# qitianwu/DIFFormer

Hardware: AMD Instinct MI355X
Metric: DIFFormer-layer forward nodes/sec (higher is better)
Workload: dtype f32; 1 GPU; ogbn-proteins-s; nodes=132534, csr_entries=79255038, in_channels=8, hidden=64, heads=1, layers=4, kernel=simple, use_graph=True, parallelism=single GPU, exact_fp32=False, csr=warm (cached), launch=eager

## Files before the change

### difformer_amd/csrc/gcn_sliced.hip

```cpp
#include <stdlib.h>
#include "dif_common.h"

namespace {

using dif::f32x4;

#ifndef DIF_SLICED_TILE_ROWS
#define DIF_SLICED_TILE_ROWS 10208
#endif
#ifndef DIF_SLICED_MAX_WAVES
#define DIF_SLICED_MAX_WAVES 16
#endif
#ifndef DIF_SLICED_WG_PER_CU
#define DIF_SLICED_WG_PER_CU 1
#endif
constexpr int kSteps = 8;
constexpr int kTileRowsMax = DIF_SLICED_TILE_ROWS;
constexpr int kLdsRows = kTileRowsMax + 16;
constexpr int kWgPerCU = DIF_SLICED_WG_PER_CU;
constexpr int kMaxRounds = 10;
constexpr int kMaxWaves = DIF_SLICED_MAX_WAVES;
constexpr int kGroupCap = 65535;

__device__ const uint8_t kLaneOf[64] = {
    0,  1,  2,  3,  12, 13, 14, 15, 20, 21, 22, 23, 24, 25, 26, 27,
    4,  5,  6,  7,  8,  9,  10, 11, 16, 17, 18, 19, 28, 29, 30, 31,
    32, 33, 34, 35, 44, 45, 46, 47, 52, 53, 54, 55, 56, 57, 58, 59,
    36, 37, 38, 39, 40, 41, 42, 43, 48, 49, 50, 51, 60, 61, 62, 63};

struct Plan {
    int slices, panels, G, PW, W, R, T, NT;
    int S = 1;
};
constexpr int kMaxSplits = 8;

__host__ __device__ __forceinline__ int64_t slot_of(int j, int pw, int PW) {
    return static_cast<int64_t>(j) * PW + ((j & 1) ? PW - 1 - pw : pw);
}

int make_plan(int64_t n_src, int64_t n_rows, int F, Plan& p) {
    if (n_src <= 0 || n_rows <= 0 || F <= 0 || F % 4 != 0 || F / 4 > 256) return DIF_E_SHAPE;
    p.slices = F / 4;
    const int64_t G = (n_rows + 63) / 64;
    int64_t panels = dif::kCUs * kWgPerCU / p.slices;
    if (panels < 1) panels = 1;
    const int64_t cap = static_cast<int64_t>(kMaxWaves) * kMaxRounds;
    if (panels * cap < G) panels = (G + cap - 1) / cap;
    const int64_t nt0 = (n_src + kTileRowsMax - 1) / kTileRowsMax;
    const int64_t need = (G + (cap - kMaxWaves) - 1) / (cap - kMaxWaves);
    int S = 1;
    while (S * 2 <= kMaxSplits && n_src + (n_src >> 4) >= int64_t(2) * S * n_rows && need * S * 2 <= panels && nt0 >= S * 2) S *= 2;
    p.S = S;
    panels /= S;
    if (panels > G) panels = G;
    if (panels * p.slices > (int64_t(1) << 20) || G >= (int64_t(1) << 30)) return DIF_E_RANGE;
    p.panels = static_cast<int>(panels);
    p.G = static_cast<int>(G);
    int bestW = 0, bestR = 1 << 30;
    int64_t bestWaste = int64_t(1) << 60;
    for (int W = kMaxWaves; W >= 1; --W) {
        const int64_t pw = panels * W;
        if (pw > G && W > 1) continue;
        const int R = static_cast<int>((G + pw - 1) / pw);
        const int64_t waste = static_cast<int64_t>(R) * pw - G;
        if (R < bestR || (R == bestR && waste < bestWaste)) { bestW = W; bestR = R; bestWaste = waste; }
    }
    if (bestR > kMaxRounds) return DIF_E_SHAPE;
    p.W = bestW;
    p.R = bestR;
    p.PW = p.panels * p.W;
    const int64_t nt = (nt0 + S - 1) / S * S;
    if (nt > 32767) return DIF_E_RANGE;
    p.NT = static_cast<int>(nt);
    p.T = static_cast<int>((((n_src + nt - 1) / nt) + 15) / 16 * 16);
    return 0;
}

__device__ __forceinline__ void group_bounds(const int32_t* __restrict__ rowptr, const int32_t* __restrict__ blkptr,
                                             int64_t n_src, int NT, int64_t row, int t, int32_t& e0, int32_t& e1) {
    if (NT == 1) { e0 = rowptr[row]; e1 = rowptr[row + 1]; }
    else { e0 = blkptr[static_cast<int64_t>(t) * n_src + row]; e1 = blkptr[static_cast<int64_t>(t + 1) * n_src + row]; }
}

__device__ __forceinline__ void position_bounds(const int32_t* __restrict__ rowptr, const int32_t* __restrict__ blkptr,
                                                int64_t n_src, int NT, int64_t row_begin, const int32_t* __restrict__ order,
                                                const uint16_t* __restrict__ parts, int64_t pos, int t, int32_t& e0,
                                                int32_t& e1) {
    const int64_t lrow = order ? order[pos] : pos;
    if (lrow < 0) { e0 = e1 = 0; return; }
    group_bounds(rowptr, blkptr, n_src, NT, row_begin + lrow, t, e0, e1);
    if (parts) {
        const uint32_t pp = parts[pos];
        const int64_t p = pp & 0xffu, P = pp >> 8, c = e1 - e0;
        e1 = e0 + static_cast<int32_t>(c * (p + 1) / P);
        e0 = e0 + static_cast<int32_t>(c * p / P);
    }
}

struct Counts { uint64_t w[4]; };

__device__ __forceinline__ Counts bucket_starts(const Counts& c) {
    const uint64_t ones = 0x0001000100010001ull;
    Counts s;
    uint64_t carry = 0;
#pragma unroll
    for (int k = 0; k < 4; ++k) {
        const uint64_t inc = c.w[k] * ones;
        s.w[k] = inc - c.w[k] + carry * ones;
        carry += inc >> 48;
    }
    return s;
}

__device__ __forceinline__ uint32_t lane16(const Counts& c, uint32_t q) {
    const uint64_t w = (q < 8u) ? ((q < 4u) ? c.w[0] : c.w[1]) : ((q < 12u) ? c.w[2] : c.w[3]);
    return static_cast<uint32_t>(w >> ((q & 3u) * 16u)) & 0xffffu;
}

__device__ __forceinline__ void bump16(Counts& c, uint32_t q) {
    const uint64_t one = 1ull << ((q & 3u) * 16u);
    const uint32_t k = q >> 2;
    c.w[0] += (k == 0u) ? one : 0ull;
    c.w[1] += (k == 1u) ? one : 0ull;
    c.w[2] += (k == 2u) ? one : 0ull;
    c.w[3] += (k == 3u) ? one : 0ull;
}

__device__ __forceinline__ Counts load_counts(const uint4* __restrict__ cnt, int64_t idx) {
    const uint4 a = cnt[idx * 2], b = cnt[idx * 2 + 1];
    Counts c;
    c.w[0] = static_cast<uint64_t>(a.x) | (static_cast<uint64_t>(a.y) << 32);
    c.w[1] = static_cast<uint64_t>(a.z) | (static_cast<uint64_t>(a.w) << 32);
    c.w[2] = static_cast<uint64_t>(b.x) | (static_cast<uint64_t>(b.y) << 32);
    c.w[3] = static_cast<uint64_t>(b.z) | (static_cast<uint64_t>(b.w) << 32);
    return c;
}

__global__ __launch_bounds__(256) void sliced_sort_kernel(const int32_t* __restrict__ rowptr, const int32_t* __restrict__ blkptr,
                                                          const int32_t* __restrict__ src, int64_t n_src, int NT, int T,
                                                          int64_t row_begin, int64_t n_pos, const int32_t* __restrict__ order,
                                                          const uint16_t* __restrict__ parts,
                                                          uint16_t* __restrict__ srt, uint4* __restrict__ cnt,
                                                          int32_t* __restrict__ status) {
    const int lane = threadIdx.x & 63;
    const int64_t pos = static_cast<int64_t>(blockIdx.x) * 4 + (threadIdx.x >> 6);
    if (pos >= n_pos) return;
    const uint64_t below = (lane == 0) ? 0ull : (~0ull >> (64 - lane));
    uint32_t* cnt32 = reinterpret_cast<uint32_t*>(cnt);
    for (int t = 0; t < NT; ++t) {
        int32_t e0, e1;
        position_bounds(rowptr, blkptr, n_src, NT, row_begin, order, parts, pos, t, e0, e1);
        e0 = __builtin_amdgcn_readfirstlane(e0);
        e1 = __builtin_amdgcn_readfirstlane(e1);
        const int32_t base = t * T;
        if (e1 - e0 > kGroupCap) {
            if (lane == 0) atomicOr(status, 1);
            e1 = e0;
        }
        uint32_t count[16];
#pragma unroll
        for (int q = 0; q < 16; ++q) count[q] = 0;
        for (int32_t c0 = e0; c0 < e1; c0 += 64) {
            const int32_t e = c0 + lane;
            const bool ok = e < e1;
            const uint32_t q = ok ? (static_cast<uint32_t>(src[e] - base) & 15u) : 16u;
#pragma unroll
            for (int qq = 0; qq < 16; ++qq) count[qq] += static_cast<uint32_t>(__popcll(__ballot(q == static_cast<uint32_t>(qq))));
        }
        uint32_t word = 0;
#pragma unroll
        for (int j = 0; j < 8; ++j)
            if (lane == j) word = count[2 * j] | (count[2 * j + 1] << 16);
        if (lane < 8) cnt32[(pos * NT + t) * 8 + lane] = word;
        uint32_t run[16];
        uint32_t acc = 0;
#pragma unroll
        for (int q = 0; q < 16; ++q) { run[q] = acc; acc += count[q]; }
        for (int32_t c0 = e0; c0 < e1; c0 += 64) {
            const int32_t e = c0 + lane;
            const bool ok = e < e1;
            const uint32_t loc = ok ? static_cast<uint32_t>(src[e] - base) : 0u;
            const uint32_t q = ok ? (loc & 15u) : 16u;
            uint32_t dst = 0;
#pragma unroll
            for (int qq = 0; qq < 16; ++qq) {
                const uint64_t m = __ballot(q == static_cast<uint32_t>(qq));
                if (q == static_cast<uint32_t>(qq)) dst = run[qq] + static_cast<uint32_t>(__popcll(m & below));
                run[qq] += static_cast<uint32_t>(__popcll(m));
            }
            if (ok) srt[e0 + dst] = static_cast<uint16_t>(loc);
        }
    }
}

constexpr int kColorThreads = 64;

template <bool EMIT>
__global__ __launch_bounds__(kColorThreads) void sliced_color_kernel(int64_t n_pos, Plan pl, int cap,
                                                                     const uint4* __restrict__ cnt,
                                                                     int32_t* __restrict__ len,
                                                                     const int32_t* __restrict__ tab,
                                                                     uint16_t* __restrict__ ell) {
    const int64_t gid = static_cast<int64_t>(blockIdx.x) * kColorThreads + threadIdx.x;
    const int64_t n_groups = static_cast<int64_t>(pl.G) * pl.NT * 4;
    if (gid >= n_groups) return;
    const int grp = static_cast<int>(gid & 3);
    const int t = static_cast<int>((gid >> 2) % pl.NT);
    const int64_t g = (gid >> 2) / pl.NT;
    const bool packed = cap > 1;
    uint32_t c[16][8];
    uint32_t col[16];
    int rem[16];
    int remaining = 0;
#pragma unroll
    for (int q = 0; q < 16; ++q) col[q] = 0;
#pragma unroll
    for (int i = 0; i < 16; ++i) {
        const int64_t pos = g * 64 + kLaneOf[grp * 16 + i];
        Counts cc = {{0, 0, 0, 0}};
        if (pos < n_pos) cc = load_counts(cnt, pos * pl.NT + t);
        rem[i] = 0;
#pragma unroll
        for (int k = 0; k < 4; ++k) {
            c[i][2 * k] = static_cast<uint32_t>(cc.w[k]);
            c[i][2 * k + 1] = static_cast<uint32_t>(cc.w[k] >> 32);
            const uint32_t q0 = cc.w[k] & 0xffffu, q1 = (cc.w[k] >> 16) & 0xffffu, q2 = (cc.w[k] >> 32) & 0xffffu,
                           q3 = static_cast<uint32_t>(cc.w[k] >> 48);
            col[4 * k] += q0; col[4 * k + 1] += q1; col[4 * k + 2] += q2; col[4 * k + 3] += q3;
            rem[i] += static_cast<int>(q0 + q1 + q2 + q3);
        }
        remaining += rem[i];
    }
    int target = 0;
    if (packed) {
        int longest = 0;
        uint32_t fullest = 0;
#pragma unroll
        for (int i = 0; i < 16; ++i) { longest = max(longest, rem[i]); fullest = max(fullest, col[i]); }
        target = max(longest, static_cast<int>((fullest + cap - 1) / cap));
        target = max(target, __shfl_xor(target, 1));
        target = max(target, __shfl_xor(target, 2));
        target = (target + kSteps - 1) / kSteps * kSteps;
    }
    const int j = static_cast<int>(g / pl.PW);
    const int idxp = static_cast<int>(g % pl.PW);
    const int pw = (j & 1) ? pl.PW - 1 - idxp : idxp;
    const int p = pw % pl.panels, w = pw / pl.panels;
    const int32_t* tb = nullptr;
    int64_t blk0 = 0;
    int nbj = 0;
    if (EMIT) {
        tb = tab + ((static_cast<int64_t>(p) * pl.NT + t) * pl.W + w) * (pl.R + 1);
        blk0 = tb[0];
        nbj = tb[1 + j];
    }
    int64_t rowbase = 0;
    auto record_at = [&](int step) -> uint4* {
        return reinterpret_cast<uint4*>(ell) + (blk0 + rowbase + j) * 64 + grp * kSteps + (step % kSteps);
    };
    auto new_row = [&](int step) {
        if (EMIT && (step % kSteps) == 0) {
            const int k = step / kSteps;
            rowbase = 0;
            for (int j2 = 0; j2 < pl.R; ++j2) { const int v = tb[1 + j2]; rowbase += v < k ? v : k; }
        }
    };
    int step = 0;
    while (remaining > 0) {
        new_row(step);
        uint32_t used = 0, full = 0, picked = 0, qlo = 0, qhi = 0;
        const int start = step & 15;
        const int left = target - step;
#pragma unroll
        for (int pass = 0; pass < 2; ++pass) {
#pragma unroll
            for (int i = 0; i < 16; ++i) {
                if ((i >= start) != (pass == 0)) continue;
                uint32_t key = 0, kshare = 0, kany = 0;
#pragma unroll
                for (int k = 0; k < 8; ++k) {
                    const uint32_t olo = c[i][k] & 0xffffu, ohi = c[i][k] >> 16;
                    const uint32_t wlo = packed ? col[2 * k] : olo, whi = packed ? col[2 * k + 1] : ohi;
                    const uint32_t lo = olo ? ((wlo << 4) | static_cast<uint32_t>(15 - 2 * k)) : 0u;
                    const uint32_t hi = ohi ? ((whi << 4) | static_cast<uint32_t>(14 - 2 * k)) : 0u;
                    const bool ulo = (used >> (2 * k)) & 1u, uhi = (used >> (2 * k + 1)) & 1u;
                    key = max(key, max(ulo ? 0u : lo, uhi ? 0u : hi));
                    if (packed) {
                        const uint32_t slo = (ulo && !((full >> (2 * k)) & 1u)) ? lo : 0u;
                        const uint32_t shi = (uhi && !((full >> (2 * k + 1)) & 1u)) ? hi : 0u;
                        kany = max(kany, max(slo, shi));
                        kshare = max(kshare, max(static_cast<int>(col[2 * k]) >= left ? slo : 0u,
                                                 static_cast<int>(col[2 * k + 1]) >= left ? shi : 0u));
                    }
                }
                bool share = false;
                if (packed) {
                    if (kshare > key) { key = kshare; share = true; }
                    else if (key < 16u && rem[i] >= left && kany >= 16u) { key = kany; share = true; }
                }
                if (key < 16u) continue;
                const uint32_t best = 15u - (key & 15u);
                if (share) full |= 1u << best;
                else used |= 1u << best;
                picked |= 1u << i;
                const uint32_t dec = 1u << (16u * (best & 1u)), wsel = best >> 1;
#pragma unroll
                for (int k = 0; k < 8; ++k) c[i][k] -= (wsel == static_cast<uint32_t>(k)) ? dec : 0u;
#pragma unroll
                for (int q = 0; q < 16; ++q) col[q] -= (best == static_cast<uint32_t>(q)) ? 1u : 0u;
                --rem[i];
                --remaining;
                if (EMIT) {
                    if (i < 8) qlo |= best << (4 * i);
                    else qhi |= best << (4 * (i - 8));
                }
            }
        }
        if (EMIT) {
#pragma unroll
            for (int i = 0; i < 16; ++i) {
                if ((picked >> i) & 1u) continue;
                const uint32_t fq = __builtin_ctz(~used & 0xffffu);
                used |= 1u << fq;
                if (i < 8) qlo |= fq << (4 * i);
                else qhi |= fq << (4 * (i - 8));
            }
            *record_at(step) = uint4{qlo, qhi, picked, 0u};
        }
        ++step;
    }
    if (!EMIT) {
        len[gid] = step;
    } else {
        for (; step < nbj * kSteps; ++step) {
            new_row(step);
            *record_at(step) = uint4{0x76543210u, 0xfedcba98u, 0u, 0u};
        }
    }
}

constexpr int kFillStage = 4096;

template <bool STAGED>
__device__ __forceinline__ void fill_blocks(const uint16_t* __restrict__ mine, const uint16_t* stage, Counts next,
                                            const int32_t* __restrict__ tb, int R, int j, int nbj, int64_t blk0, int grp,
                                            int i, int lane, uint32_t T, uint4* __restrict__ ell) {
    uint64_t n0 = next.w[0], n1 = next.w[1], n2 = next.w[2], n3 = next.w[3];
    const uint32_t himask = (i >= 8) ? ~0u : 0u, sh = 4u * (i & 7);
    for (int k = 0; k < nbj; ++k) {
        int64_t rowbase = 0;
        for (int j2 = 0; j2 < R; ++j2) { const int v = tb[1 + j2]; rowbase += v < k ? v : k; }
        uint4* blk = ell + (blk0 + rowbase + j) * 64;
        uint4 rec[kSteps];
#pragma unroll
        for (int s8 = 0; s8 < kSteps; ++s8) rec[s8] = blk[grp * kSteps + s8];
        uint32_t ent[kSteps];
#pragma unroll
        for (int s8 = 0; s8 < kSteps; ++s8) {
            const uint32_t q = ((((rec[s8].x & ~himask) | (rec[s8].y & himask)) >> sh)) & 15u;
            const bool real = (rec[s8].z >> i) & 1u;
            const uint32_t k = q >> 2;
            const uint64_t m0 = k == 0u ? ~0ull : 0ull, m1 = k == 1u ? ~0ull : 0ull, m2 = k == 2u ? ~0ull : 0ull,
                           m3 = k == 3u ? ~0ull : 0ull;
            const uint64_t wsel = (n0 & m0) | (n1 & m1) | (n2 & m2) | (n3 & m3);
            const uint32_t qs = (q & 3u) * 16u;
            const uint32_t at = real ? (static_cast<uint32_t>(wsel >> qs) & 0xffffu) : 0u;
            const uint32_t v = STAGED ? stage[at] : mine[at];
            const uint64_t one = real ? (1ull << qs) : 0ull;
            n0 += one & m0; n1 += one & m1; n2 += one & m2; n3 += one & m3;
            ent[s8] = real ? v : T + q;
        }
        blk[lane] = uint4{ent[0] | (ent[1] << 16), ent[2] | (ent[3] << 16), ent[4] | (ent[5] << 16), ent[6] | (ent[7] << 16)};
    }
}

__global__ __launch_bounds__(256) void sliced_fill_kernel(
    const int32_t* __restrict__ rowptr, const int32_t* __restrict__ blkptr, int64_t n_src, int64_t row_begin,
    int64_t n_pos, const int32_t* __restrict__ order, const uint16_t* __restrict__ parts, Plan pl,
    const uint16_t* __restrict__ srt, const uint4* __restrict__ cnt, const int32_t* __restrict__ tab,
    uint4* __restrict__ ell) {
    __shared__ uint16_t stage_s[4][kFillStage + 8];
    const int lane = threadIdx.x & 63;
    const int wave = threadIdx.x >> 6;
    const int64_t gw = static_cast<int64_t>(blockIdx.x) * 4 + wave;
    const int64_t g = gw / pl.NT;
    const int t = static_cast<int>(gw % pl.NT);
    if (g >= pl.G) return;
    const int j = static_cast<int>(g / pl.PW);
    const int idxp = static_cast<int>(g % pl.PW);
    const int pw = (j & 1) ? pl.PW - 1 - idxp : idxp;
    const int p = pw % pl.panels, w = pw / pl.panels;
    const int32_t* tb = tab + ((static_cast<int64_t>(p) * pl.NT + t) * pl.W + w) * (pl.R + 1);
    const int64_t blk0 = tb[0];
    const int nbj = tb[1 + j];
    if (nbj == 0) return;
    int inv = 0;
#pragma unroll
    for (int k = 0; k < 64; ++k) inv = (kLaneOf[k] == lane) ? k : inv;
    const int grp = inv >> 4, i = inv & 15;
    const int64_t pos = g * 64 + lane;
    Counts next = {{0, 0, 0, 0}};
    int32_t e0 = 0, e1 = 0;
    if (pos < n_pos) {
        position_bounds(rowptr, blkptr, n_src, pl.NT, row_begin, order, parts, pos, t, e0, e1);
        next = bucket_starts(load_counts(cnt, pos * pl.NT + t));
    }
    const int mycnt = e1 - e0;
    int inc = mycnt;
#pragma unroll
    for (int o = 1; o < 64; o <<= 1) {
        const int v = __shfl_up(inc, o, 64);
        if (lane >= o) inc += v;
    }
    const int total = __shfl(inc, 63, 64);
    uint16_t* stage = stage_s[wave];
    if (total <= kFillStage) {
        const int off = inc - mycnt;
        for (int r0 = 0; r0 < 64; r0 += 16) {
            uint16_t v[16];
#pragma unroll
            for (int u = 0; u < 16; ++u) {
                const int n_r = __builtin_amdgcn_readlane(mycnt, r0 + u);
                const int32_t e_r = __builtin_amdgcn_readlane(e0, r0 + u);
                v[u] = (lane < n_r) ? srt[e_r + lane] : uint16_t(0);
            }
#pragma unroll
            for (int u = 0; u < 16; ++u) {
                const int n_r = __builtin_amdgcn_readlane(mycnt, r0 + u), off_r = __builtin_amdgcn_readlane(off, r0 + u);
                if (lane < n_r) stage[off_r + lane] = v[u];
            }
            for (int u = 0; u < 16; ++u) {
                const int n_r = __builtin_amdgcn_readlane(mycnt, r0 + u), off_r = __builtin_amdgcn_readlane(off, r0 + u);
                const int32_t e_r = __builtin_amdgcn_readlane(e0, r0 + u);
                for (int x = lane + 64; x < n_r; x += 64) stage[off_r + x] = srt[e_r + x];
            }
        }
        __builtin_amdgcn_wave_barrier();
        fill_blocks<true>(nullptr, stage + off, next, tb, pl.R, j, nbj, blk0, grp, i, lane, static_cast<uint32_t>(pl.T),
                          ell);
    } else {
        fill_blocks<false>(mycnt > 0 ? srt + e0 : srt, nullptr, next, tb, pl.R, j, nbj, blk0, grp, i, lane,
                           static_cast<uint32_t>(pl.T), ell);
    }
}

__global__ __launch_bounds__(1024) void sliced_table_kernel(const int32_t* __restrict__ len, Plan pl, int32_t* __restrict__ tab) {
    __shared__ int32_t sm[1024];
    __shared__ int32_t carry;
    const int64_t n = static_cast<int64_t>(pl.panels) * pl.NT * pl.W;
    if (threadIdx.x == 0) carry = 0;
    __syncthreads();
    for (int64_t base = 0; base < n; base += 1024) {
        const int64_t idx = base + threadIdx.x;
        int32_t blocks = 0;
        if (idx < n) {
            const int w = static_cast<int>(idx % pl.W);
            const int t = static_cast<int>((idx / pl.W) % pl.NT);
            const int p = static_cast<int>(idx / pl.W / pl.NT);
            const int pw = w * pl.panels + p;
            int32_t* row = tab + idx * (pl.R + 1);
            int32_t env = 0;
            for (int j = pl.R - 1; j >= 0; --j) {
                const int64_t g = slot_of(j, pw, pl.PW);
                int32_t nb = 0;
                if (g < pl.G) {
                    for (int q = 0; q < 4; ++q) {
                        const int32_t v = (len[(g * pl.NT + t) * 4 + q] + kSteps - 1) / kSteps;
                        nb = v > nb ? v : nb;
                    }
                }
                env = nb > env ? nb : env;
                row[1 + j] = env;
                blocks += env;
            }
        }
        sm[threadIdx.x] = blocks;
        __syncthreads();
        for (int off = 1; off < 1024; off <<= 1) {
            const int32_t tv = (static_cast<int>(threadIdx.x) >= off) ? sm[threadIdx.x - off] : 0;
            __syncthreads();
            sm[threadIdx.x] += tv;
            __syncthreads();
        }
        const int32_t cin = carry;
        if (idx < n) tab[idx * (pl.R + 1)] = cin + sm[threadIdx.x] - blocks;
        __syncthreads();
        if (threadIdx.x == 1023) carry = cin + sm[1023];
        __syncthreads();
    }
    if (threadIdx.x == 0) tab[n * (pl.R + 1)] = carry;
}

__device__ __forceinline__ float dinv_of(const int32_t* __restrict__ rowptr, int64_t row) {
    const int32_t d = rowptr[row + 1] - rowptr[row];
    return d > 0 ? sqrtf(1.0f / static_cast<float>(d)) : 0.f;
}

constexpr int kPreSlices = 32;

__global__ __launch_bounds__(256) void sliced_prescale_kernel(const float* __restrict__ x, int64_t ldx,
                                                              const int32_t* __restrict__ rowptr,
                                                              const float* __restrict__ dinv, int64_t n_src,
                                                              int64_t npad, int slices, f32x4* __restrict__ ys) {
    __shared__ f32x4 stage[kPreSlices * 65];
    const int64_t row0 = static_cast<int64_t>(blockIdx.x) * 64;
    const int s0 = blockIdx.y * kPreSlices;
    const int ns = (slices - s0 < kPreSlices) ? slices - s0 : kPreSlices;
    const int total = 64 * ns;
    for (int e = threadIdx.x; e < total; e += 256) {
        const int r = e / ns, sl = e % ns;
        const int64_t row = row0 + r;
        f32x4 v = f32x4{0.f, 0.f, 0.f, 0.f};
        if (row < n_src)
            v = *reinterpret_cast<const f32x4*>(x + row * ldx + (s0 + sl) * 4) * (dinv ? dinv[row] : dinv_of(rowptr, row));
        stage[sl * 65 + r] = v;
    }
    __syncthreads();
    for (int e = threadIdx.x; e < total; e += 256) {
        const int sl = e / 64, r = e % 64;
        const int64_t row = row0 + r;
        if (row < npad) ys[static_cast<int64_t>(s0 + sl) * npad + row] = stage[sl * 65 + r];
    }
}

struct Epilogue {
    const int32_t* rowptr;
    const float* dinv;
    const int32_t* order;
    const uint16_t* parts;
    int64_t row_begin, n_pos;
    const float* attn;
    int64_t lda;
    float attn_scale, gcn_scale;
    float* out;
    int64_t ldo;
    f32x4* partial;
};

__device__ __forceinline__ f32x4 add4(f32x4 x, f32x4 y) {
    return x + y;
}

__device__ __forceinline__ void block8(const f32x4* tile, uint4& e, const uint4* reload, f32x4& a) {
    const uint32_t four = 4;
    const uint32_t wds[4] = {e.x, e.y, e.z, e.w};
    uint32_t ad[8];
#pragma unroll
    for (int q = 0; q < 4; ++q) {
        asm("v_lshlrev_b32_sdwa %0, %1, %2 dst_sel:DWORD dst_unused:UNUSED_PAD src0_sel:DWORD src1_sel:WORD_0"
            : "=v"(ad[2 * q]) : "v"(four), "v"(wds[q]));
        asm("v_lshlrev_b32_sdwa %0, %1, %2 dst_sel:DWORD dst_unused:UNUSED_PAD src0_sel:DWORD src1_sel:WORD_1"
            : "=v"(ad[2 * q + 1]) : "v"(four), "v"(wds[q]));
    }
    e = *reload;
    f32x4 v[4];
#pragma unroll
    for (int q = 0; q < 4; ++q) v[q] = *reinterpret_cast<const f32x4*>(reinterpret_cast<const char*>(tile) + ad[q]);
    a = add4(a, add4(add4(v[0], v[1]), add4(v[2], v[3])));
#pragma unroll
    for (int q = 0; q < 4; ++q) v[q] = *reinterpret_cast<const f32x4*>(reinterpret_cast<const char*>(tile) + ad[4 + q]);
    a = add4(a, add4(add4(v[0], v[1]), add4(v[2], v[3])));
}

template <int M, int NR>
struct Phases {
    static __device__ __forceinline__ void run(const f32x4* tile, int& k, const uint4*& cur, uint4 (&e)[NR], f32x4 (&acc)[NR],
                                               const int (&nb)[NR]) {
        const int kend = nb[M - 1];
#pragma unroll 1
        for (; k + 1 < kend; ++k) {
            const uint4* nx = cur + M * 64;
#pragma unroll
            for (int j = 0; j < M; ++j) {
                block8(tile, e[j], nx + j * 64, acc[j]);
                __builtin_amdgcn_sched_barrier(0);
            }
            cur = nx;
        }
        if (k < kend) {
            const uint4* nx = cur + M * 64;
#pragma unroll
            for (int j = 0; j < M; ++j) {
                block8(tile, e[j], (nb[j] > k + 1) ? nx + j * 64 : cur, acc[j]);
                __builtin_amdgcn_sched_barrier(0);
            }
            cur = nx;
            ++k;
            __builtin_amdgcn_s_waitcnt(0x0F70);
        }
        Phases<M - 1, NR>::run(tile, k, cur, e, acc, nb);
    }
};
template <int NR>
struct Phases<0, NR> {
    static __device__ __forceinline__ void run(const f32x4*, int&, const uint4*&, uint4 (&)[NR], f32x4 (&)[NR], const int (&)[NR]) {}
};

__device__ __forceinline__ void finish_position(const Epilogue& ep, int64_t pos, int slice, f32x4 acc) {
    int64_t lrow = -1;
    if (pos < ep.n_pos) lrow = ep.order ? ep.order[pos] : pos;
    f32x4 sum = acc;
    if (ep.parts) {
        const uint32_t pp = (pos < ep.n_pos && lrow >= 0) ? ep.parts[pos] : 0x0100u;
        const int p = pp & 0xffu, P = pp >> 8;
        for (int k = 1; __ballot(k < P) != 0ull; ++k) {
            f32x4 o;
            o.x = __shfl_down(acc.x, k);
            o.y = __shfl_down(acc.y, k);
            o.z = __shfl_down(acc.z, k);
            o.w = __shfl_down(acc.w, k);
            if (p == 0 && k < P) sum += o;
        }
        if (p != 0) lrow = -1;
    }
    if (lrow >= 0) {
        const int64_t row = ep.row_begin + lrow;
        f32x4 o = sum * (ep.gcn_scale * (ep.dinv ? ep.dinv[row] : dinv_of(ep.rowptr, row)));
        if (ep.attn) o += ep.attn_scale * *reinterpret_cast<const f32x4*>(ep.attn + lrow * ep.lda + slice * 4);
        *reinterpret_cast<f32x4*>(ep.out + lrow * ep.ldo + slice * 4) = o;
    }
}

template <int NR>
__device__ __forceinline__ void sweep(f32x4* tile, const uint4* __restrict__ ell, const int32_t* __restrict__ tabw,
                                      int64_t tab_stride, const f32x4* __restrict__ ysl, const Plan pl, const Epilogue ep,
                                      int pw, int slice, int lane, int t0, int z) {
    constexpr int NA = NR > 0 ? NR : 1;
    const int T = pl.T;
    f32x4 acc[NA];
#pragma unroll
    for (int j = 0; j < NA; ++j) acc[j] = f32x4{0.f, 0.f, 0.f, 0.f};
    const int ntl = pl.NT / pl.S;
    for (int tt = 0; tt < ntl; ++tt) {
        int t = tt + t0;
        if (t >= ntl) t -= ntl;
        t += z * ntl;
        uint4 e[NA];
        int nb[NA];
        const uint4* cur = ell;
        if (NR > 0) {
            const int32_t* tr = tabw + static_cast<int64_t>(t) * tab_stride;
            cur = ell + static_cast<int64_t>(__builtin_amdgcn_readfirstlane(tr[0])) * 64 + lane;
#pragma unroll
            for (int j = 0; j < NR; ++j) {
                nb[j] = __builtin_amdgcn_readfirstlane(tr[1 + j]);
                e[j] = *((nb[j] > 0) ? cur + j * 64 : ell);
            }
        }
        {
            constexpr int U = NR >= 10 ? 4 : (NR == 9 ? 7 : (NR == 8 ? 9 : 11));
            const f32x4* src = ysl + static_cast<int64_t>(t) * T;
            const int nth = blockDim.x;
            const uint32_t tid = threadIdx.x;
            f32x4 r[U];
#pragma unroll
            for (int u = 0; u < U; ++u) {
                const f32x4* su = src + u * nth;
                r[u] = (u * nth + static_cast<int>(tid) < T) ? su[tid] : f32x4{0.f, 0.f, 0.f, 0.f};
            }
            __syncthreads();
#pragma unroll
            for (int b = 0; b < 11; b += U) {
#pragma unroll
                for (int u = 0; u < U; ++u) {
                    if (b + u < 11) {
                        f32x4* du = tile + (b + u) * nth;
                        if ((b + u) * nth + static_cast<int>(tid) < T) du[tid] = r[u];
                    }
                    if (b + U + u < 11) {
                        const f32x4* su = src + (b + U + u) * nth;
                        r[u] = ((b + U + u) * nth + static_cast<int>(tid) < T) ? su[tid] : f32x4{0.f, 0.f, 0.f, 0.f};
                    }
                }
            }
            for (int b0 = static_cast<int>(tid) + 11 * nth; b0 < T; b0 += nth) tile[b0] = src[b0];
        }
        __builtin_amdgcn_s_waitcnt(0x0F70);
        __syncthreads();
        if (NR > 0) {
            int k = 0;
            Phases<NR, NA>::run(tile, k, cur, e, acc, nb);
        }
    }
#pragma unroll
    for (int j = 0; j < NR; ++j) {
        const int64_t pos = slot_of(j, pw, pl.PW) * 64 + lane;
        if (pl.S > 1) ep.partial[(static_cast<int64_t>(z) * pl.slices + slice) * pl.G * 64 + pos] = acc[j];
        else finish_position(ep, pos, slice, acc[j]);
    }
}

template <int R>
__global__ __launch_bounds__(64 * kMaxWaves, (kWgPerCU * kMaxWaves + 3) / 4) void sliced_spmm_kernel(const uint4* __restrict__ ell, const int32_t* __restrict__ tab,
                                                                     const f32x4* __restrict__ ys, int64_t npad, Plan pl,
                                                                     Epilogue ep) {
    __shared__ f32x4 tile[kLdsRows];
    const int b = blockIdx.x;
    int vp, slice, t0 = 0;
    const int per = gridDim.x >> 3;
    if ((gridDim.x & 7) == 0 && per % pl.slices == 0) {
        const int xcd = b & 7, k = b >> 3;
        vp = xcd * (per / pl.slices) + k / pl.slices;
        slice = k % pl.slices;
        t0 = (xcd * (pl.NT / pl.S)) >> 3;
    } else {
        vp = b / pl.slices;
        slice = b % pl.slices;
    }
    const int panel = vp / pl.S, z = vp % pl.S;
    const int lane = threadIdx.x & 63;
    const int w = __builtin_amdgcn_readfirstlane(threadIdx.x >> 6);
    if (threadIdx.x < 16) tile[pl.T + threadIdx.x] = f32x4{0.f, 0.f, 0.f, 0.f};
    const f32x4* ysl = ys + static_cast<int64_t>(slice) * npad;
    const int32_t* tabw = tab + (static_cast<int64_t>(panel) * pl.NT * pl.W + w) * (pl.R + 1);
    const int64_t tab_stride = static_cast<int64_t>(pl.W) * (pl.R + 1);
    const int pw = w * pl.panels + panel;
    const bool full = slot_of(R - 1, pw, pl.PW) < pl.G;
    if (full) sweep<R>(tile, ell, tabw, tab_stride, ysl, pl, ep, pw, slice, lane, t0, z);
    else sweep<R - 1>(tile, ell, tabw, tab_stride, ysl, pl, ep, pw, slice, lane, t0, z);
}

__global__ __launch_bounds__(256) void sliced_combine_kernel(Plan pl, Epilogue ep) {
    const int64_t pair = static_cast<int64_t>(blockIdx.x) * 4 + (threadIdx.x >> 6);
    if (pair >= static_cast<int64_t>(pl.G) * pl.slices) return;
    const int slice = static_cast<int>(pair % pl.slices);
    const int64_t pos = (pair / pl.slices) * 64 + (threadIdx.x & 63);
    const int64_t plane = static_cast<int64_t>(pl.G) * 64;
    const f32x4* src = ep.partial + slice * plane + pos;
    f32x4 v[kMaxSplits];
#pragma unroll
    for (int z = 0; z < kMaxSplits; ++z)
        if (z < pl.S) v[z] = src[static_cast<int64_t>(z) * pl.slices * plane];
    f32x4 sum = v[0];
#pragma unroll
    for (int z = 1; z < kMaxSplits; ++z)
        if (z < pl.S) sum += v[z];
    finish_position(ep, pos, slice, sum);
}

template <int R>
int launch_sweep(hipStream_t st, const uint4* ell, const int32_t* tab, const f32x4* ys, int64_t npad, const Plan& pl,
                 const Epilogue& ep) {
    hipLaunchKernelGGL((sliced_spmm_kernel<R>), dim3(static_cast<unsigned>(pl.panels * pl.S * pl.slices)), dim3(64 * pl.W),
                       0, st, ell, tab, ys, npad, pl, ep);
    if (int rc = dif::launch_status("sliced_spmm_kernel")) return rc;
    if (pl.S == 1) return 0;
    const int64_t pairs = static_cast<int64_t>(pl.G) * pl.slices;
    hipLaunchKernelGGL(sliced_combine_kernel, dim3(static_cast<unsigned>((pairs + 3) / 4)), dim3(256), 0, st, pl, ep);
    return dif::launch_status("sliced_combine_kernel");
}

int check_positions(const int32_t* row_order, const uint16_t* parts, int64_t n_rows, int64_t n_pos, const char* who) {
    if (parts ? (row_order == nullptr || n_pos < n_rows) : (n_pos != n_rows))
        return dif::fail(DIF_E_BADARG, "%s: n_pos must equal n_rows without `parts`; with `parts`, row_order and n_pos >= "
                         "n_rows are required", who);
    return 0;
}

constexpr int32_t kPlanSlicesMask = 0xffff, kPlanCapMask = 0x30000;
int plan_quad_cap(const int32_t* plan) { return ((plan[0] & kPlanCapMask) >> 16) + 1; }

int check_plan(const int32_t* plan, int64_t n_src, int64_t n_rows, int F, Plan& pl) {
    if (!plan) return dif::fail(DIF_E_BADARG, "dif_sliced: plan is null");
    Plan want;
    const int rc = make_plan(n_src, n_rows, F, want);
    if (rc) return dif::fail(rc, "dif_sliced: shape not covered (n_src=%lld, n_rows=%lld, F=%d)",
                             static_cast<long long>(n_src), static_cast<long long>(n_rows), F);
    pl = Plan{plan[0] & kPlanSlicesMask, plan[1], plan[2], plan[3], plan[4], plan[5], plan[6], plan[7], want.S};
    if ((plan[0] & ~(kPlanSlicesMask | kPlanCapMask)) != 0) pl.slices = -1;
    if (pl.slices != want.slices || pl.panels != want.panels || pl.G != want.G || pl.PW != want.PW || pl.W != want.W ||
        pl.R != want.R || pl.T != want.T || pl.NT != want.NT)
        return dif::fail(DIF_E_BADARG, "dif_sliced: plan does not match dif_sliced_plan(n_src, n_rows, F)");
    return 0;
}

}

extern "C" int dif_sliced_plan(int64_t n_src, int64_t n_rows, int F, int32_t* plan) {
    DIF_REQUIRE(plan != nullptr, DIF_E_BADARG, "dif_sliced_plan: plan is null");
    Plan p;
    const int rc = make_plan(n_src, n_rows, F, p);
    if (rc) return dif::fail(rc, "dif_sliced_plan: shape not covered (n_src=%lld, n_rows=%lld, F=%d): needs F %% 4 == 0, "
                             "F <= 1024", static_cast<long long>(n_src), static_cast<long long>(n_rows), F);
    const int32_t v[8] = {p.slices, p.panels, p.G, p.PW, p.W, p.R, p.T, p.NT};
    for (int i = 0; i < 8; ++i) plan[i] = v[i];
    return 0;
}

extern "C" int64_t dif_sliced_spmm_workspace_bytes(int64_t n_src, int64_t n_rows, int F) {
    Plan p;
    if (make_plan(n_src, n_rows, F, p) != 0 || p.S == 1) return 0;
    return static_cast<int64_t>(p.S) * p.slices * p.G * 64 * 16;
}

extern "C" int dif_sliced_measure(const int32_t* rowptr, const int32_t* blkptr, const int32_t* src, int64_t n_src,
                                  int64_t nnz, int64_t row_begin, int64_t n_rows, int F, const int32_t* plan,
                                  const int32_t* row_order, const uint16_t* parts, int64_t n_pos, uint16_t* sorted,
                                  void* counts, int32_t* lengths, int32_t* table, int32_t* status, dif_stream_t stream) {
    Plan pl;
    if (int rc = check_positions(row_order, parts, n_rows, n_pos, "dif_sliced_measure")) return rc;
    if (int rc = check_plan(plan, n_src, n_pos, F, pl)) return rc;
    const int quad_cap = plan_quad_cap(plan);
    DIF_REQUIRE(quad_cap <= 2, DIF_E_BADARG, "dif_sliced_measure: the plan's quad capacity must be 1 (strict) or 2 (packed)");
    DIF_REQUIRE(row_begin >= 0 && row_begin + n_rows <= n_src && nnz >= 0, DIF_E_BADARG, "dif_sliced_measure: bad row range");
    DIF_REQUIRE(rowptr && (nnz == 0 || src) && sorted && counts && lengths && table && status, DIF_E_BADARG,
                "dif_sliced_measure: null pointer");
    DIF_REQUIRE(pl.NT == 1 || blkptr, DIF_E_BADARG,
                "dif_sliced_measure: more than one tile needs the CSR built with n_blocks = plan[7], block_rows = plan[6]");
    DIF_REQUIRE(dif::aligned16(counts), DIF_E_BADARG, "dif_sliced_measure: counts must be 16-byte aligned");
    hipStream_t st = static_cast<hipStream_t>(stream);
    hipError_t he = hipMemsetAsync(status, 0, 4, st);
    if (he != hipSuccess) return dif::fail(static_cast<int>(he), "dif_sliced_measure: memset: %s", hipGetErrorString(he));
    hipLaunchKernelGGL(sliced_sort_kernel, dim3(static_cast<unsigned>((n_pos + 3) / 4)), dim3(256), 0, st, rowptr,
                       blkptr, src, n_src, pl.NT, pl.T, row_begin, n_pos, row_order, parts, sorted,
                       static_cast<uint4*>(counts), status);
    if (int rc = dif::launch_status("sliced_sort_kernel")) return rc;
    const int64_t n_hw = static_cast<int64_t>(pl.G) * pl.NT * 4;
    hipLaunchKernelGGL((sliced_color_kernel<false>), dim3(static_cast<unsigned>((n_hw + kColorThreads - 1) / kColorThreads)),
                       dim3(kColorThreads), 0, st, n_pos, pl, quad_cap, static_cast<const uint4*>(counts), lengths, nullptr,
                       nullptr);
    if (int rc = dif::launch_status("sliced_color_kernel")) return rc;
    hipLaunchKernelGGL(sliced_table_kernel, dim3(1), dim3(1024), 0, st, lengths, pl, table);
    return dif::launch_status("sliced_table_kernel");
}

extern "C" int dif_sliced_emit(const int32_t* rowptr, const int32_t* blkptr, int64_t n_src, int64_t row_begin,
                               int64_t n_rows, int F, const int32_t* plan, const int32_t* row_order, const uint16_t* parts,
                               int64_t n_pos, const uint16_t* sorted, const void* counts, const int32_t* table,
                               int64_t n_blocks, uint16_t* entries, dif_stream_t stream) {
    Plan pl;
    if (int rc = check_positions(row_order, parts, n_rows, n_pos, "dif_sliced_emit")) return rc;
    if (int rc = check_plan(plan, n_src, n_pos, F, pl)) return rc;
    const int quad_cap = plan_quad_cap(plan);
    DIF_REQUIRE(quad_cap <= 2, DIF_E_BADARG, "dif_sliced_emit: the plan's quad capacity must be 1 (strict) or 2 (packed)");
    DIF_REQUIRE(rowptr && sorted && counts && table && entries && n_blocks >= 1, DIF_E_BADARG, "dif_sliced_emit: null pointer");
    DIF_REQUIRE(pl.NT == 1 || blkptr, DIF_E_BADARG, "dif_sliced_emit: more than one tile needs blkptr");
    DIF_REQUIRE(dif::aligned16(entries) && dif::aligned16(counts), DIF_E_BADARG,
                "dif_sliced_emit: entries / counts must be 16-byte aligned");
    hipStream_t st = static_cast<hipStream_t>(stream);
    const int64_t n_hw = static_cast<int64_t>(pl.G) * pl.NT * 4;
    hipLaunchKernelGGL((sliced_color_kernel<true>), dim3(static_cast<unsigned>((n_hw + kColorThreads - 1) / kColorThreads)),
                       dim3(kColorThreads), 0, st, n_pos, pl, quad_cap, static_cast<const uint4*>(counts), nullptr, table,
                       entries);
    if (int rc = dif::launch_status("sliced_color_kernel")) return rc;
    const int64_t n_st = static_cast<int64_t>(pl.G) * pl.NT;
    hipLaunchKernelGGL(sliced_fill_kernel, dim3(static_cast<unsigned>((n_st + 3) / 4)), dim3(256), 0, st, rowptr, blkptr,
                       n_src, row_begin, n_pos, row_order, parts, pl, sorted, static_cast<const uint4*>(counts), table,
                       reinterpret_cast<uint4*>(entries));
    return dif::launch_status("sliced_fill_kernel");
}

extern "C" int dif_sliced_prescale_f32(const float* x, int64_t ldx, const int32_t* rowptr, const float* dinv, int64_t n_src,
                                       int F, const int32_t* plan, float* ys, dif_stream_t stream) {
    DIF_REQUIRE(x && rowptr && plan && ys && n_src > 0 && F > 0 && F % 4 == 0 && ldx >= F, DIF_E_BADARG,
                "dif_sliced_prescale: bad argument");
    DIF_REQUIRE(ldx % 4 == 0 && dif::aligned16(x) && dif::aligned16(ys), DIF_E_BADARG,
                "dif_sliced_prescale: x rows and ys must be 16-byte aligned");
    const int slices = plan[0] & kPlanSlicesMask;
    const int64_t npad = static_cast<int64_t>(plan[6]) * plan[7];
    DIF_REQUIRE(slices == F / 4 && npad >= n_src, DIF_E_BADARG, "dif_sliced_prescale: plan does not match F / n_src");
    hipStream_t st = static_cast<hipStream_t>(stream);
    hipLaunchKernelGGL(sliced_prescale_kernel, dim3(static_cast<unsigned>((npad + 63) / 64), (slices + kPreSlices - 1) / kPreSlices),
                       dim3(256), 0, st, x, ldx, rowptr, dinv, n_src, npad, slices, reinterpret_cast<f32x4*>(ys));
    return dif::launch_status("sliced_prescale_kernel");
}

extern "C" int dif_sliced_spmm_f32(const uint16_t* entries, const int32_t* table, const int32_t* plan, const float* ys,
                                   const int32_t* rowptr, const float* dinv, const int32_t* row_order, const uint16_t* parts,
                                   int64_t n_pos, int64_t n_src, int64_t row_begin, int64_t n_rows, int F, const float* attn,
                                   int64_t lda, float attn_scale, float gcn_scale, float* out, int64_t ldo, void* ws,
                                   int64_t ws_bytes, dif_stream_t stream) {
    Plan pl;
    if (int rc = check_positions(row_order, parts, n_rows, n_pos, "dif_sliced_spmm")) return rc;
    if (int rc = check_plan(plan, n_src, n_pos, F, pl)) return rc;
    const int64_t ws_need = pl.S > 1 ? static_cast<int64_t>(pl.S) * pl.slices * pl.G * 64 * 16 : 0;
    DIF_REQUIRE(ws_need == 0 || (ws && ws_bytes >= ws_need && dif::aligned16(ws)), DIF_E_BADARG,
                "dif_sliced_spmm: a row shard's product needs dif_sliced_spmm_workspace_bytes() of 16-byte aligned workspace");
    DIF_REQUIRE(entries && table && ys && rowptr && out, DIF_E_BADARG, "dif_sliced_spmm: null pointer");
    DIF_REQUIRE(row_begin >= 0 && row_begin + n_rows <= n_src, DIF_E_BADARG, "dif_sliced_spmm: row range exceeds n_src");
    DIF_REQUIRE(ldo >= F && ldo % 4 == 0 && dif::aligned16(out) && (!attn || (lda >= F && lda % 4 == 0 && dif::aligned16(attn))),
                DIF_E_BADARG, "dif_sliced_spmm: out / attn rows must be 16-byte aligned with ld >= F");
    DIF_REQUIRE(dif::aligned16(entries) && dif::aligned16(ys), DIF_E_BADARG, "dif_sliced_spmm: entries / ys must be 16-byte aligned");
    hipStream_t st = static_cast<hipStream_t>(stream);
    const int64_t npad = static_cast<int64_t>(pl.T) * pl.NT;
    const Epilogue ep = {rowptr, dinv, row_order, parts, row_begin, n_pos, attn, lda, attn_scale, gcn_scale, out, ldo,
                         static_cast<f32x4*>(ws)};
    const uint4* e4 = reinterpret_cast<const uint4*>(entries);
    const f32x4* y4 = reinterpret_cast<const f32x4*>(ys);
    switch (pl.R) {
        case 1: return launch_sweep<1>(st, e4, table, y4, npad, pl, ep);
        case 2: return launch_sweep<2>(st, e4, table, y4, npad, pl, ep);
        case 3: return launch_sweep<3>(st, e4, table, y4, npad, pl, ep);
        case 4: return launch_sweep<4>(st, e4, table, y4, npad, pl, ep);
        case 5: return launch_sweep<5>(st, e4, table, y4, npad, pl, ep);
        case 6: return launch_sweep<6>(st, e4, table, y4, npad, pl, ep);
        case 7: return launch_sweep<7>(st, e4, table, y4, npad, pl, ep);
        case 8: return launch_sweep<8>(st, e4, table, y4, npad, pl, ep);
        case 9: return launch_sweep<9>(st, e4, table, y4, npad, pl, ep);
        case 10: return launch_sweep<10>(st, e4, table, y4, npad, pl, ep);
    }
    return dif::fail(DIF_E_SHAPE, "dif_sliced_spmm: %d rounds per wave not covered", pl.R);
}
```

Baseline: 90.90 million nodes/s.

## Rebalance last-round ELL rows across waves by lending rounds between SIMD groups

Adds a host-computed lending plan in which fully loaded waves hand their last ELL round to less loaded waves on lighter SIMD lanes (wave index mod 4), so per-SIMD work is balanced within a workgroup. Borrowers run the extra round with a separate accumulator, reading the donor's table entries and strided ELL rows, and write results to the donor's output slot. This targets imbalance where some SIMDs idle while others finish an extra round. It adds more kernel template instantiations, host-side planning on every launch (including a getenv call), and more register pressure from the extra accumulators.

```diff
diff --git a/difformer_amd/csrc/gcn_sliced.hip b/difformer_amd/csrc/gcn_sliced.hip
--- a/difformer_amd/csrc/gcn_sliced.hip
+++ b/difformer_amd/csrc/gcn_sliced.hip
@@ -562,32 +562,37 @@
     a = add4(a, add4(add4(v[0], v[1]), add4(v[2], v[3])));
 }
 
+template <int M, int ST, int NR>
+__device__ __forceinline__ void phase_rows(const f32x4* tile, int& k, const uint4*& cur, uint4 (&e)[NR], f32x4 (&acc)[NR],
+                                           const int (&nb)[NR], const int kend) {
+#pragma unroll 1
+    for (; k + 1 < kend; ++k) {
+        const uint4* nx = cur + ST * 64;
+#pragma unroll
+        for (int j = 0; j < M; ++j) {
+            block8(tile, e[j], nx + j * 64, acc[j]);
+            __builtin_amdgcn_sched_barrier(0);
+        }
+        cur = nx;
+    }
+    if (k < kend) {
+        const uint4* nx = cur + ST * 64;
+#pragma unroll
+        for (int j = 0; j < M; ++j) {
+            block8(tile, e[j], (nb[j] > k + 1) ? nx + j * 64 : cur, acc[j]);
+            __builtin_amdgcn_sched_barrier(0);
+        }
+        cur = nx;
+        ++k;
+        __builtin_amdgcn_s_waitcnt(0x0F70);
+    }
+}
+
 template <int M, int NR>
 struct Phases {
     static __device__ __forceinline__ void run(const f32x4* tile, int& k, const uint4*& cur, uint4 (&e)[NR], f32x4 (&acc)[NR],
                                                const int (&nb)[NR]) {
-        const int kend = nb[M - 1];
-#pragma unroll 1
-        for (; k + 1 < kend; ++k) {
-            const uint4* nx = cur + M * 64;
-#pragma unroll
-            for (int j = 0; j < M; ++j) {
-                block8(tile, e[j], nx + j * 64, acc[j]);
-                __builtin_amdgcn_sched_barrier(0);
-            }
-            cur = nx;
-        }
-        if (k < kend) {
-            const uint4* nx = cur + M * 64;
-#pragma unroll
-            for (int j = 0; j < M; ++j) {
-                block8(tile, e[j], (nb[j] > k + 1) ? nx + j * 64 : cur, acc[j]);
-                __builtin_amdgcn_sched_barrier(0);
-            }
-            cur = nx;
-            ++k;
-            __builtin_amdgcn_s_waitcnt(0x0F70);
-        }
+        phase_rows<M, M, NR>(tile, k, cur, e, acc, nb, nb[M - 1]);
         Phases<M - 1, NR>::run(tile, k, cur, e, acc, nb);
     }
 };
@@ -621,15 +626,44 @@
     }
 }
 
-template <int NR>
+template <int NE>
+__device__ __forceinline__ void borrowed_round(const f32x4* tile, const uint4* ell_lane, const int64_t first, const int R,
+                                               const int nbd, uint4 (&e)[NE], f32x4& a) {
+    const uint4* nxt = ell_lane + first * 64;
+    int left = nbd;
+#pragma unroll
+    for (int i = 0; i < NE; ++i) {
+        e[i] = *((left > 0) ? nxt : ell_lane);
+        nxt += R * 64;
+        --left;
+    }
+#pragma unroll 1
+    for (int k0 = 0; k0 < nbd; k0 += NE) {
+#pragma unroll
+        for (int i = 0; i < NE; ++i) {
+            if (k0 + i < nbd) {
+                block8(tile, e[i], (left > 0) ? nxt : ell_lane, a);
+                __builtin_amdgcn_sched_barrier(0);
+                nxt += R * 64;
+                --left;
+            }
+        }
+    }
+    __builtin_amdgcn_s_waitcnt(0x0F70);
+}
+
+template <int NR, int NB, bool LENT>
 __device__ __forceinline__ void sweep(f32x4* tile, const uint4* __restrict__ ell, const int32_t* __restrict__ tabw,
                                       int64_t tab_stride, const f32x4* __restrict__ ysl, const Plan pl, const Epilogue ep,
-                                      int pw, int slice, int lane, int t0, int z) {
+                                      int pw, int slice, int lane, int t0, int z, const int donors) {
     constexpr int NA = NR > 0 ? NR : 1;
+    constexpr int NBA = NB > 0 ? NB : 1;
     const int T = pl.T;
-    f32x4 acc[NA];
+    f32x4 acc[NA], accb[NBA];
 #pragma unroll
     for (int j = 0; j < NA; ++j) acc[j] = f32x4{0.f, 0.f, 0.f, 0.f};
+#pragma unroll
+    for (int i = 0; i < NBA; ++i) accb[i] = f32x4{0.f, 0.f, 0.f, 0.f};
     const int ntl = pl.NT / pl.S;
     for (int tt = 0; tt < ntl; ++tt) {
         int t = tt + t0;
@@ -648,7 +682,8 @@
             }
         }
         {
-            constexpr int U = NR >= 10 ? 4 : (NR == 9 ? 7 : (NR == 8 ? 9 : 11));
+            constexpr int NT_ = NR + NB;
+            constexpr int U = NT_ >= 10 ? 4 : (NT_ == 9 ? 7 : (NT_ == 8 ? 9 : 11));
             const f32x4* src = ysl + static_cast<int64_t>(t) * T;
             const int nth = blockDim.x;
             const uint32_t tid = threadIdx.x;
@@ -679,7 +714,16 @@
         __syncthreads();
         if (NR > 0) {
             int k = 0;
+            if (LENT)
+                phase_rows<NR, NR + 1, NA>(tile, k, cur, e, acc, nb,
+                                           __builtin_amdgcn_readfirstlane(tabw[static_cast<int64_t>(t) * tab_stride + 1 + NR]));
             Phases<NR, NA>::run(tile, k, cur, e, acc, nb);
+        }
+#pragma unroll
+        for (int i = 0; i < NB; ++i) {
+            const int32_t* td = tabw + static_cast<int64_t>(t) * tab_stride + static_cast<int8_t>(donors >> (8 * i)) * (pl.R + 1);
+            const int64_t first = __builtin_amdgcn_readfirstlane(td[0]) + (pl.R - 1);
+            borrowed_round<NA>(tile, ell + lane, first, pl.R, __builtin_amdgcn_readfirstlane(td[pl.R]), e, accb[i]);
         }
     }
 #pragma unroll
@@ -688,12 +732,73 @@
         if (pl.S > 1) ep.partial[(static_cast<int64_t>(z) * pl.slices + slice) * pl.G * 64 + pos] = acc[j];
         else finish_position(ep, pos, slice, acc[j]);
     }
+#pragma unroll
+    for (int i = 0; i < NB; ++i) {
+        const int64_t pos = slot_of(pl.R - 1, pw + static_cast<int8_t>(donors >> (8 * i)) * pl.panels, pl.PW) * 64 + lane;
+        if (pl.S > 1) ep.partial[(static_cast<int64_t>(z) * pl.slices + slice) * pl.G * 64 + pos] = accb[i];
+        else finish_position(ep, pos, slice, accb[i]);
+    }
+}
+
+struct Lend {
+    int nfull_min;
+    uint32_t rec[2][kMaxWaves];
+};
+
+__host__ __device__ __forceinline__ int full_waves(const Plan& pl, int panel) {
+    int n = 0;
+    for (int w = 0; w < pl.W; ++w) n += slot_of(pl.R - 1, w * pl.panels + panel, pl.PW) < pl.G ? 1 : 0;
+    return n;
+}
+
+void make_lend(const Plan& pl, bool on, Lend& ld) {
+    ld.nfull_min = pl.W;
+    for (int k = 0; k < 2; ++k)
+        for (int w = 0; w < kMaxWaves; ++w) ld.rec[k][w] = 0;
+    for (int p = 0; p < pl.panels; ++p) { const int n = full_waves(pl, p); if (n < ld.nfull_min) ld.nfull_min = n; }
+    if (!on) return;
+    for (int k = 0; k < 2; ++k) {
+        int p = 0;
+        while (p < pl.panels && full_waves(pl, p) != ld.nfull_min + k) ++p;
+        if (p == pl.panels) continue;
+        bool full[kMaxWaves];
+        int accs[kMaxWaves], nbor[kMaxWaves], load[4] = {0, 0, 0, 0};
+        for (int w = 0; w < pl.W; ++w) {
+            full[w] = slot_of(pl.R - 1, w * pl.panels + p, pl.PW) < pl.G;
+            accs[w] = full[w] ? pl.R : pl.R - 1;
+            nbor[w] = 0;
+            load[w & 3] += accs[w];
+        }
+        uint32_t* rec = ld.rec[k];
+        for (;;) {
+            int lo = 0;
+            for (int g = 1; g < 4 && g < pl.W; ++g) if (load[g] < load[lo]) lo = g;
+            int hi = -1;
+            for (int g = 0; g < 4; ++g) {
+                if (hi < 0 || load[g] > load[hi]) { hi = g; continue; }
+                if (load[g] == load[hi] && (hi ^ lo) == 2 && (g ^ lo) != 2) hi = g;
+            }
+            if (load[hi] - load[lo] < 2) break;
+            int donor = -1, borrower = -1;
+            for (int w = hi; w < pl.W; w += 4) if (full[w] && !(rec[w] & 1u) && nbor[w] == 0) donor = w;
+            for (int w = lo; w < pl.W; w += 4)
+                if (!(rec[w] & 1u) && nbor[w] < (full[w] ? 1 : 2) && accs[w] < kMaxRounds && (borrower < 0 || accs[w] < accs[borrower]))
+                    borrower = w;
+            if (donor < 0 || borrower < 0) break;
+            rec[donor] |= 1u | static_cast<uint32_t>(borrower + 1) << 24;
+            rec[borrower] += (1u << 4) + (static_cast<uint32_t>(donor) << (8 + 8 * nbor[borrower]));
+            ++nbor[borrower];
+            ++accs[borrower];
+            --load[hi];
+            ++load[lo];
+        }
+    }
 }
 
 template <int R>
 __global__ __launch_bounds__(64 * kMaxWaves, (kWgPerCU * kMaxWaves + 3) / 4) void sliced_spmm_kernel(const uint4* __restrict__ ell, const int32_t* __restrict__ tab,
                                                                      const f32x4* __restrict__ ys, int64_t npad, Plan pl,
-                                                                     Epilogue ep) {
+                                                                     Epilogue ep, Lend lend, uint32_t* __restrict__ lend_out) {
     __shared__ f32x4 tile[kLdsRows];
     const int b = blockIdx.x;
     int vp, slice, t0 = 0;
@@ -716,8 +821,24 @@
     const int64_t tab_stride = static_cast<int64_t>(pl.W) * (pl.R + 1);
     const int pw = w * pl.panels + panel;
     const bool full = slot_of(R - 1, pw, pl.PW) < pl.G;
-    if (full) sweep<R>(tile, ell, tabw, tab_stride, ysl, pl, ep, pw, slice, lane, t0, z);
-    else sweep<R - 1>(tile, ell, tabw, tab_stride, ysl, pl, ep, pw, slice, lane, t0, z);
+    const uint32_t rec = lend.rec[full_waves(pl, panel) > lend.nfull_min ? 1 : 0][w];
+    if (lend_out && slice == 0 && z == 0 && lane == 0) lend_out[panel * pl.W + w] = rec;
+    const bool lent = rec & 1u;
+    const uint32_t nbor = (rec >> 4) & 15u;
+    const int donors = static_cast<int>(((((rec >> 8) & 255u) - w) & 255u) | (((((rec >> 16) & 255u) - w) & 255u) << 8));
+#define DIF_SWEEP(NR, NB, LENT) sweep<NR, NB, LENT>(tile, ell, tabw, tab_stride, ysl, pl, ep, pw, slice, lane, t0, z, donors)
+    if (nbor == 0) {
+        if (!full) DIF_SWEEP(R - 1, 0, false);
+        else if (!lent) DIF_SWEEP(R, 0, false);
+        else DIF_SWEEP(R - 1, 0, true);
+    } else if (full) {
+        if constexpr (R + 1 <= kMaxRounds) DIF_SWEEP(R, 1, false);
+    } else if (nbor == 1) {
+        DIF_SWEEP(R - 1, 1, false);
+    } else {
+        DIF_SWEEP(R - 1, 2, false);
+    }
+#undef DIF_SWEEP
 }
 
 __global__ __launch_bounds__(256) void sliced_combine_kernel(Plan pl, Epilogue ep) {
@@ -740,9 +861,12 @@
 
 template <int R>
 int launch_sweep(hipStream_t st, const uint4* ell, const int32_t* tab, const f32x4* ys, int64_t npad, const Plan& pl,
-                 const Epilogue& ep) {
+                 const Epilogue& ep, uint32_t* lend_out) {
+    const char* sw = getenv("DIFFORMER_SLICED_LEND");
+    Lend lend;
+    make_lend(pl, !(sw && sw[0] == '0'), lend);
     hipLaunchKernelGGL((sliced_spmm_kernel<R>), dim3(static_cast<unsigned>(pl.panels * pl.S * pl.slices)), dim3(64 * pl.W),
-                       0, st, ell, tab, ys, npad, pl, ep);
+                       0, st, ell, tab, ys, npad, pl, ep, lend, lend_out);
     if (int rc = dif::launch_status("sliced_spmm_kernel")) return rc;
     if (pl.S == 1) return 0;
     const int64_t pairs = static_cast<int64_t>(pl.G) * pl.slices;
@@ -887,17 +1011,20 @@
                          static_cast<f32x4*>(ws)};
     const uint4* e4 = reinterpret_cast<const uint4*>(entries);
     const f32x4* y4 = reinterpret_cast<const f32x4*>(ys);
+    const int64_t lend_bytes = static_cast<int64_t>(pl.panels) * pl.W * 4;
+    uint32_t* lo = (ws && ws_bytes >= ws_need + lend_bytes && dif::aligned16(ws))
+                       ? reinterpret_cast<uint32_t*>(static_cast<char*>(ws) + ws_need) : nullptr;
     switch (pl.R) {
-        case 1: return launch_sweep<1>(st, e4, table, y4, npad, pl, ep);
-        case 2: return launch_sweep<2>(st, e4, table, y4, npad, pl, ep);
-        case 3: return launch_sweep<3>(st, e4, table, y4, npad, pl, ep);
-        case 4: return launch_sweep<4>(st, e4, table, y4, npad, pl, ep);
-        case 5: return launch_sweep<5>(st, e4, table, y4, npad, pl, ep);
-        case 6: return launch_sweep<6>(st, e4, table, y4, npad, pl, ep);
-        case 7: return launch_sweep<7>(st, e4, table, y4, npad, pl, ep);
-        case 8: return launch_sweep<8>(st, e4, table, y4, npad, pl, ep);
-        case 9: return launch_sweep<9>(st, e4, table, y4, npad, pl, ep);
-        case 10: return launch_sweep<10>(st, e4, table, y4, npad, pl, ep);
+        case 1: return launch_sweep<1>(st, e4, table, y4, npad, pl, ep, lo);
+        case 2: return launch_sweep<2>(st, e4, table, y4, npad, pl, ep, lo);
+        case 3: return launch_sweep<3>(st, e4, table, y4, npad, pl, ep, lo);
+        case 4: return launch_sweep<4>(st, e4, table, y4, npad, pl, ep, lo);
+        case 5: return launch_sweep<5>(st, e4, table, y4, npad, pl, ep, lo);
+        case 6: return launch_sweep<6>(st, e4, table, y4, npad, pl, ep, lo);
+        case 7: return launch_sweep<7>(st, e4, table, y4, npad, pl, ep, lo);
+        case 8: return launch_sweep<8>(st, e4, table, y4, npad, pl, ep, lo);
+        case 9: return launch_sweep<9>(st, e4, table, y4, npad, pl, ep, lo);
+        case 10: return launch_sweep<10>(st, e4, table, y4, npad, pl, ep, lo);
     }
     return dif::fail(DIF_E_SHAPE, "dif_sliced_spmm: %d rounds per wave not covered", pl.R);
 }
```

After: 85.67 million nodes/s. -5.8%, worse.
